# bluemoon-o2/walker-gym

Hardware: AMD Instinct MI355X
Metric: env-steps/sec (whole node) at 65 536 walkers; 1/2/4/8 MI355X scaling (higher is better)
Workload: dtype f32

## Files before the change

include/walker_hip.h:

```cpp
#ifndef WALKER_HIP_H
#define WALKER_HIP_H
#include <stdint.h>

#ifdef __cplusplus
extern "C" {
#endif

typedef struct ihipStream_t *hipStream_t;
typedef struct ihipEvent_t *hipEvent_t;

#define WG_ABI_VERSION 16
#define WG_EINVAL (-1)
#define WG_ERANGE (-2)
#define WG_EHIP (-3)

typedef struct wg_params {
    double g, dampk, ground, groundk, grounddamp, friction, dt;
    double pk, vk, ak, mk;
    int32_t in3d, max_steps;
    int32_t midform;
    int32_t conmid;
    int32_t spring_mode;
    int32_t action_mode;
    int32_t integrator;
// ... 124 lines not shown
               int32_t plan_blocks, hipStream_t stream);

typedef wg_params wg_obs_cfg;
int wg_step_simple(const wg_batch *b, const float *action, const wg_params *p, int32_t n_steps, hipStream_t stream);
int wg_observe_simple(const wg_batch *b, const wg_obs_cfg *cfg, float *obs, float *reward, uint8_t *done,
                      float *centroid, float *energy, hipStream_t stream);

int wg_reset(const wg_batch *b, const wg_params *p, const float *noise, const uint8_t *mask,
             hipStream_t stream);

int wg_reset_noise(const wg_batch *b, const float *noise, hipStream_t stream);

int wg_plan_ragged(const int32_t *mass_off, const int32_t *edge_off, const int32_t *muscle_off,
                   int32_t N, int32_t *plan, int32_t max_blocks);

int wg_plan_waves(const int32_t *mass_off, const int32_t *edge_off, const int32_t *muscle_off,
                  int32_t N, int32_t *plan, int32_t max_tiles);
int wg_wave_edge_passes(int32_t M, int32_t K);

int wg_plan_errors(int32_t clear);

int wg_launch_geometry(const wg_batch *b, wg_launch_info *info);

int wg_debug_stamps(unsigned long long *host, int n);

int wg_launch_floor(int32_t mode, int32_t blocks, int32_t threads, const float *in, float *out, int32_t n_launches,
                    hipStream_t stream);

int wg_time_step(const wg_batch *batch, const wg_params *params, const float *action, int32_t action_cols,
                 int32_t action_stride, int64_t action_step, const wg_outputs *out, int32_t n_steps,
                 const int32_t *plan, int32_t plan_blocks, hipStream_t stream, float *ms_per_launch);

#ifdef __cplusplus
}
#endif
#endif
```

walker_gym_amd/_lib.py:

```python
from __future__ import annotations

import ctypes as C
import os
import threading

HERE = os.path.dirname(os.path.abspath(__file__))
LIB_NAME = "libwalker_hip.so"
LIB_PATH = os.path.join(HERE, LIB_NAME)
ABI_VERSION = 16

WG_EINVAL, WG_ERANGE, WG_EHIP = -1, -2, -3

_vp = C.c_void_p


class WgParams(C.Structure):
    _fields_ = [(n, C.c_double) for n in ("g", "dampk", "ground", "groundk", "grounddamp", "friction", "dt",
                                           "pk", "vk", "ak", "mk")] + \
               [(n, C.c_int32) for n in ("in3d", "max_steps", "midform", "conmid", "spring_mode", "action_mode",
                                         "integrator", "pair_mode")] + \
               [(n, C.c_double) for n in ("pair_g", "pair_k", "pair_e", "bounce_k")] + \
               [("g3_gravity", C.c_double * 3)] + \
               [(n, C.c_double) for n in ("g3_damping", "g3_air", "g3_ground_level", "g3_restitution",
                                          "g3_friction")] + [("g3_ground", C.c_int32), ("friction_mode", C.c_int32),
# ... 27 lines not shown
    _fields_ = [("batch", C.POINTER(WgBatch)), ("outputs", C.POINTER(WgOutputs)), ("action_offset", C.c_int64),
                ("plan", _vp), ("plan_blocks", C.c_int32), ("stream", _vp)]


class WgLaunchInfo(C.Structure):
    _fields_ = [("threads", C.c_int32), ("walkers_per_block", C.c_int32), ("blocks", C.c_int32),
                ("lds_bytes", C.c_int32)]


class WgPolicy(C.Structure):
    _fields_ = [("n_sets", C.c_int32), ("obs_dim", C.c_int32), ("hidden", C.c_int32), ("act_dim", C.c_int32),
                ("w1", _vp), ("b1", _vp), ("w2", _vp), ("b2", _vp), ("act_limit", C.c_float),
                ("action_out", _vp), ("action_out_step", C.c_int64), ("return_out", _vp), ("length_out", _vp)]


class WgEpisodeStats(C.Structure):
    _fields_ = [("return_sum", _vp), ("length_sum", _vp), ("episodes_done", _vp), ("tail_return", _vp),
                ("tail_length", _vp), ("ep_return", _vp), ("ep_length", _vp), ("ep_slots", C.c_int32)]


EXPORTS = ("wg_abi_version", "wg_last_error", "wg_step", "wg_step_ranges", "wg_run_ranges", "wg_rollout", "wg_observe",
           "wg_step_simple", "wg_observe_simple", "wg_reset", "wg_reset_noise", "wg_plan_ragged", "wg_plan_waves",
           "wg_wave_edge_passes", "wg_plan_errors", "wg_launch_geometry", "wg_launch_floor", "wg_time_step",
           "wg_rollout_policy", "wg_rollout_episodes")

_lib = None
_lock = threading.Lock()


class WalkerHipError(RuntimeError):
    pass


def load(path: str | None = None):
    global _lib
    with _lock:
        if _lib is not None:
            return _lib
        p = path or os.environ.get("WALKER_HIP_LIB", LIB_PATH)
        if not os.path.exists(p):
            raise WalkerHipError(
                f"{p} not found: build it with `python -m walker_gym_amd.build` (hipcc --offload-arch=gfx950); "
                "walker_gym_amd has no CPU fallback")
        L = C.CDLL(p)
        L.wg_abi_version.restype = C.c_int
        L.wg_last_error.restype = C.c_char_p
        L.wg_step.argtypes = [C.POINTER(WgBatch), C.POINTER(WgParams), _vp, C.c_int32, C.c_int32, C.c_int64,
# ... 1 lines not shown
        L.wg_rollout.argtypes = L.wg_step.argtypes
        L.wg_rollout_policy.argtypes = [C.POINTER(WgBatch), C.POINTER(WgParams), C.POINTER(WgPolicy),
                                        C.POINTER(WgOutputs), C.c_int32, _vp]
        L.wg_rollout_episodes.argtypes = [C.POINTER(WgBatch), C.POINTER(WgParams), C.POINTER(WgPolicy),
                                          C.POINTER(WgOutputs), C.POINTER(WgEpisodeStats), C.c_int32, _vp]
        L.wg_step_ranges.argtypes = [C.POINTER(WgRange), C.c_int32, C.POINTER(WgParams), _vp, C.c_int32, C.c_int32,
                                     C.POINTER(_vp)]
        L.wg_run_ranges.argtypes = [C.POINTER(WgRange), C.c_int32, C.POINTER(WgParams), _vp, C.c_int32, C.c_int32,
                                    C.c_int64, C.c_int32, C.POINTER(_vp)]
        L.wg_observe.argtypes = [C.POINTER(WgBatch), C.POINTER(WgParams), C.POINTER(WgOutputs), _vp, C.c_int32, _vp]
        L.wg_step_simple.argtypes = [C.POINTER(WgBatch), _vp, C.POINTER(WgParams), C.c_int32, _vp]
        L.wg_observe_simple.argtypes = [C.POINTER(WgBatch), C.POINTER(WgParams), _vp, _vp, _vp, _vp, _vp, _vp]
        L.wg_reset.argtypes = [C.POINTER(WgBatch), C.POINTER(WgParams), _vp, _vp, _vp]
        L.wg_reset_noise.argtypes = [C.POINTER(WgBatch), _vp, _vp]
        L.wg_plan_ragged.argtypes = [_vp, _vp, _vp, C.c_int32, _vp, C.c_int32]
        L.wg_plan_waves.argtypes = [_vp, _vp, _vp, C.c_int32, _vp, C.c_int32]
        L.wg_wave_edge_passes.argtypes = [C.c_int32, C.c_int32]
        L.wg_plan_errors.argtypes = [C.c_int32]
        L.wg_launch_geometry.argtypes = [C.POINTER(WgBatch), C.POINTER(WgLaunchInfo)]
        L.wg_launch_floor.argtypes = [C.c_int32, C.c_int32, C.c_int32, _vp, _vp, C.c_int32, _vp]
        L.wg_time_step.argtypes = L.wg_step.argtypes + [C.POINTER(C.c_float)]
        for f in EXPORTS[2:]:
            getattr(L, f).restype = C.c_int
        v = L.wg_abi_version()
        if v != ABI_VERSION:
            raise WalkerHipError(f"{p}: ABI version {v}, expected {ABI_VERSION}")
        _lib = L
        return L


def check(rc: int, what: str) -> int:
    if rc < 0:
        msg = load().wg_last_error().decode(errors="replace")
        exc = ValueError if rc in (WG_EINVAL, WG_ERANGE) else WalkerHipError
        raise exc(f"{what}: {msg} (code {rc})")
    return rc
```

walker_gym_amd/csrc/walker_hip.hip:

```cpp

#include <hip/hip_runtime.h>
#include <hip/hip_ext.h>

#include <algorithm>
#include <cstdarg>
#include <cstdint>
#include <cstdio>
#include <cstdlib>
#include <cstring>
#include <type_traits>
#include <vector>

#include "walker_hip.h"
#include "powf2.h"

namespace {

thread_local char g_err[512] = "";

int fail(int code, const char *fmt, ...) __attribute__((format(printf, 2, 3)));
int fail(int code, const char *fmt, ...) {
    va_list ap;
    va_start(ap, fmt);
    vsnprintf(g_err, sizeof g_err, fmt, ap);
    va_end(ap);
    return code;
}
// ... 1567 lines not shown
    spring_terms(e, x, pix, piy, piz, pjx, pjy, pjz, vix, viy, viz, vjx, vjy, vjz, t0, t1, t2, g0, g1, g2, spring_mode,
                 pos_ok);
    ts.put(le, t0, t1, t2, g0, g1, g2);
    gt = gt || fexp3(g0, g1, g2) < TINY_EXP;
}

struct EdgeRec8 { uint32_t w; float rest; };
template <int NE, bool E8 = false>
struct LeanIn {
    float p3[3], v3[3];
    typename std::conditional<E8, EdgeRec8, EdgeRec>::type er[NE];
    uint32_t gi[NE];
    float mf;
    int io0, io1, wsteps, pin;
    float x, lo, hi, stp, a;
};

struct LeanTile {
    int w0, nw, nP, nE, nU, wl, q, mu_wl, mu_ua;
    uint32_t P0, E0, U0;
    bool is_mass, is_mus, acts;
};

__device__ __forceinline__ LeanTile lean_tile_of(const wg_batch &b, const float *action, int action_cols,
                                                 const LeanGeo &lg, int tile, int lane) {
    LeanTile t;
    t.w0 = tile * lg.wpw;
    t.nw = min(lg.wpw, b.N - t.w0);
    t.nP = t.nw * b.M; t.nE = t.nw * b.K; t.nU = t.nw * b.A;
    t.P0 = (uint32_t)t.w0 * b.M; t.E0 = (uint32_t)t.w0 * b.K; t.U0 = (uint32_t)t.w0 * b.A;
    t.wl = lane >> lg.lgM; t.q = lane & (b.M - 1);
    t.is_mass = lane < t.nP;
    t.is_mus = lane < t.nU;
    t.mu_wl = b.A > 0 ? fdiv(lane, b.A, lg.invA) : 0;
    t.mu_ua = lane - t.mu_wl * b.A;
    t.acts = action != nullptr && t.is_mus && t.mu_ua < action_cols;
    return t;
}

template <typename T>
__device__ __forceinline__ const T &at_u32(const T *base, uint32_t byte_off) {
    return *reinterpret_cast<const T *>(reinterpret_cast<const char *>(base) + (size_t)byte_off);
}
template <typename T>
__device__ __forceinline__ T &at_u32w(T *base, uint32_t byte_off) {
    return *reinterpret_cast<T *>(reinterpret_cast<char *>(base) + (size_t)byte_off);
}
#define WG_ST(base, e, n) (&at_u32w((base), (uint32_t)(n) * 4u * (uint32_t)(e)))
__device__ __forceinline__ float neg_half_count(int n) { return -0.5f * (float)n; }
template <class LI>
__device__ __forceinline__ void lean_load_mass(const wg_batch &b, const LeanTile &t, int lane, LI &L) {
    L.mf = 0.f; L.io0 = 0; L.io1 = 0; L.wsteps = 0; L.pin = 0;
    const int ln = min(lane, t.nP - 1);
    const int wl = ln >> (31 - __builtin_clz(b.M)), q = ln & (b.M - 1);
    L.mf = at_u32(b.mass, 4u * (t.P0 + ln));
    if (b.pinned) L.pin = at_u32(b.pinned, t.P0 + ln);
    const uint32_t io = (uint32_t)(t.w0 + wl) * (b.M + 1) + q;
    L.io0 = at_u32(b.inc_off, 2u * io); L.io1 = at_u32(b.inc_off, 2u * io + 2u);
    L.wsteps = at_u32(b.steps, 4u * (uint32_t)(t.w0 + wl));
}
template <class LI>
__device__ __forceinline__ void lean_load_muscles(const wg_batch &b, const KParams &kp, const float *__restrict__ action,
                                                  int action_stride, const LeanTile &t, int lane, LI &L) {
    L.x = 0.f; L.lo = 0.f; L.hi = 0.f; L.stp = 0.f; L.a = 0.f;
    if (t.nU > 0) {
        const uint32_t ul = t.U0 + min(lane, t.nU - 1);
        L.x = at_u32(b.muscle_x, 4u * ul);
        if (action && action_stride > 0) {
            const float2 bd = at_u32(reinterpret_cast<const float2 *>(b.muscle_bounds), 8u * ul);
            L.lo = bd.x; L.hi = bd.y;
            if (kp.action_mode == 1) L.stp = at_u32(b.muscle_stride, 4u * ul);
            const int wl = min(t.mu_wl, t.nw - 1), ua = max(0, min(t.mu_ua, action_stride - 1));
            L.a = at_u32(action, 4u * ((uint32_t)(t.w0 + wl) * (uint32_t)action_stride + (uint32_t)ua));
        }
    }
}
template <int NE, bool E8>
__device__ __forceinline__ void lean_load(const wg_batch &b, const KParams &kp, const float *__restrict__ action,
                                          int action_stride, const LeanTile &t, int lane, LeanIn<NE, E8> &L) {
    const uint32_t pl = t.P0 + min(lane, t.nP - 1);
    const float *gp = &at_u32(b.pos, 12u * pl), *gv = &at_u32(b.vel, 12u * pl);
    L.p3[0] = gp[0]; L.p3[1] = gp[1]; L.p3[2] = gp[2];
    L.v3[0] = gv[0]; L.v3[1] = gv[1]; L.v3[2] = gv[2];
#pragma unroll
    for (int it = 0; it < NE; it++) {
        const uint32_t le = t.E0 + (uint32_t)min(lane + 64 * it, t.nE - 1);
        if constexpr (E8) {
            const uint2 v = at_u32(reinterpret_cast<const uint2 *>(b.edges8), 8u * le);
            L.er[it] = EdgeRec8{v.x, __uint_as_float(v.y)};
        } else {
            const uint4 v = at_u32(reinterpret_cast<const uint4 *>(b.edges), 16u * le);
            L.er[it] = EdgeRec{v.x, __uint_as_float(v.y), __uint_as_float(v.z), __uint_as_float(v.w)};
        }
        L.gi[it] = at_u32(reinterpret_cast<const uint32_t *>(b.inc), 4u * le);
    }
    lean_load_mass(b, t, lane, L);
    lean_load_muscles(b, kp, action, action_stride, t, lane, L);
    if (!t.is_mass) {
        L.p3[0] = 0.f; L.p3[1] = 0.f; L.p3[2] = 0.f; L.v3[0] = 0.f; L.v3[1] = 0.f; L.v3[2] = 0.f;
        L.mf = 0.f; L.pin = 0; L.io0 = 0; L.io1 = 0;
    }
    if (!t.is_mus) { L.x = 0.f; L.lo = 0.f; L.hi = 0.f; L.stp = 0.f; }
// ... 135 lines not shown
    if (kp.pair_mode & 2) {
        const double e = (b.charge && is_mass) ? b.charge[pl] : kp.pair_e;
        pair_central(kp.pair_k, e, p3, mf, lane, M, is_mass, ax, ay, az);
    }
    if (kp.pair_mode & 4) {
        const double rs = is_mass ? b.radius[pl] : 0.0;
        const int bs = b.bounce_set ? (is_mass ? (int)b.bounce_set[pl] : 0) : 3;
        pair_bounce(kp.bounce_kh, rs, bs, p3, mf, lane, M, is_mass, ax, ay, az);
    }
    if (kp.pair_mode & 8) pair_g2_gravity(kp.pair_g, p3, mf, lane, M, is_mass, ax, ay, az);
    if (kp.pair_mode & 16) {
        const double e = (b.charge && is_mass) ? b.charge[pl] : kp.pair_e;
        pair_central(kp.pair_k, e, p3, mf, lane, M, is_mass, ax, ay, az, true);
    }
}



typedef TermsAoS LeanTerms;
__device__ __forceinline__ LeanTerms lean_terms(char *sl, const LeanGeo &lg) {
    return TermsAoS{reinterpret_cast<double *>(sl), reinterpret_cast<float *>(sl + lg.off_df)};
}

template <bool IN3D>
__device__ __forceinline__ void lean_obs_rows(float *obs, int stride, const KParams &kp, int M, int A, int w0, int wl,
                                              int q, int mu_wl, int mu_ua, bool mass_on, bool mus_on, float px, float py,
                                              float pz, float vx, float vy, float vz, float ax, float ay, float az,
                                              float sx, float sy, float sz, float midx, float midy, float midz, float x) {
    constexpr int d = IN3D ? 3 : 2, per = 3 * d;
    const int nmid = kp.conmid ? 3 : 0;
    typedef float fvd __attribute__((ext_vector_type(d), aligned(4)));
    if (mass_on) {
        const uint32_t row0 = (uint32_t)(w0 + wl) * (uint32_t)stride;
        const float mm[3] = {kp.midform == 2 ? sx : midx, kp.midform == 2 ? sy : midy, kp.midform == 2 ? sz : midz};
        const float pm[3] = {px, py, pz}, vm[3] = {vx, vy, vz}, am[3] = {ax, ay, az};
        fvd vp, vv, va;
#pragma unroll
        for (int c = 0; c < d; c++) {
            vp[c] = kp.midform ? (pm[c] - mm[c]) * kp.pk : pm[c] * kp.pk;
            vv[c] = vm[c] * kp.vk;
            va[c] = am[c] * kp.ak;
        }
        float *dst = WG_ST(obs, row0 + per * q, 1);
        *reinterpret_cast<fvd *>(dst) = vp;
        *reinterpret_cast<fvd *>(dst + d) = vv;
        *reinterpret_cast<fvd *>(dst + 2 * d) = va;
        if (q == 0) {
            if (nmid) {
                float *mrow = WG_ST(obs, row0 + per * M, 1);
                mrow[0] = kp.midform ? mm[0] : 0.f; mrow[1] = kp.midform ? mm[1] : 0.f;
                mrow[2] = kp.midform ? mm[2] : 0.f;
            }
            for (int r = per * M + nmid + A; r < stride; r++) *WG_ST(obs, row0 + r, 1) = 0.f;
        }
    }
    if (mus_on) *WG_ST(obs, (uint32_t)(w0 + mu_wl) * (uint32_t)stride + per * M + nmid + mu_ua, 1) = x * kp.mk;
}

struct LeanPolOut { float ax, ay, az, sx, sy, sz, reward; int done; int reset; };
template <bool IN3D, int NE, bool RES = false, bool E8 = false, bool AR = false, bool POL = false>
__device__ __forceinline__ void lean_compute(const wg_batch &b, const KParams &kp, const KOut &o,
                                             const LeanGeo &lg, char *sl, const LeanTile &t, int lane,
                                             LeanIn<NE, E8> &L, bool last = true, const KReset &ar = KReset{},
                                             LeanPolOut *po = nullptr, uint32_t *epw = nullptr, int epw_stride = 1) {
    const bool store = !RES || last;
    const int M = b.M, K = b.K, A = b.A;
    const int w0 = t.w0, nE = t.nE;
    const int wl = t.wl, q = t.q, mu_wl = t.mu_wl, mu_ua = t.mu_ua;
    const bool is_mass = t.is_mass, is_mus = t.is_mus, acts = t.acts;
    const uint32_t pl = t.P0 + lane, ul = t.U0 + lane;
    const LeanTerms ts = lean_terms(sl, lg);
#ifdef WG_STAMPS
    const int stamp_wave = t.w0 / lg.wpw;
#endif
    uint32_t *s_inc = reinterpret_cast<uint32_t *>(sl + lg.off_inc);
    float *s_x = reinterpret_cast<float *>(sl + lg.off_x);
    const float mf = L.mf;
    const bool pin = L.pin != 0;
    double sq_tl = 0.0, sq_te = 0.0;
    if (NE == 1 && !RES) {
        sq_tl = PW_LOG2_TAB[lane & 31];
        sq_te = pw_asdouble(PW_EXP2_TAB[lane & 31]);
    }

    if (!RES) {
#pragma unroll
        for (int it = 0; it < NE; it++)
            if (lane + 64 * it < nE) s_inc[lane + 64 * it] = L.gi[it];
        if (lane == 0) s_inc[nE] = 0u;
    }
    float x = L.x;
    if (acts) {
        x = (kp.action_mode == 1) ? ((L.a != 0.f) ? x + L.stp : x - L.stp) : x + L.a;
        if (L.lo > x) x = L.lo;
        if (L.hi < x) x = L.hi;
        if (store) *WG_ST(b.muscle_x, ul, 1) = x;
    }
    if (is_mus) s_x[lane] = x;
    double ym = recip_m(mf);
    if (!RES) asm volatile("" : "+v"(ym));
    wave_sync();
    STAMP(2);

    bool dead = false;
    if ((!RES || NE == 1) && kp.pair_mode == 0) {
        const bool nanp = is_mass && (__builtin_isnan(L.p3[0]) || __builtin_isnan(L.p3[1]) || __builtin_isnan(L.p3[2]));
        if (__builtin_expect(__ballot(nanp) != 0ull, 0)) {
            const unsigned long long db = __ballot(nanp && !pin && L.io1 > L.io0);
            const unsigned long long gm = (M == 64) ? ~0ull : (((1ull << M) - 1ull) << (lane & ~(M - 1)));
            dead = is_mass && (db & gm) == gm;
            if (dead) {
// ... 24 lines not shown
                continue;
            }
            g.v[c] = lane_gather(L.p3[c], bi); g.v[3 + c] = lane_gather(L.p3[c], bj);
            g.v[6 + c] = lane_gather(L.v3[c], bi); g.v[9 + c] = lane_gather(L.v3[c], bj);
        }
    };
    auto spring = [&](int it, const Gath &g) {
        const int le = lane + 64 * it;
        EdgeRec e;
        float xr;
        if constexpr (E8) {
            const uint32_t w = L.er[it].w;
            const bool mus = (w & 0x40000000u) != 0u;
            const float xs = *reinterpret_cast<const float *>(reinterpret_cast<const char *>(s_x) + ((w >> 16) & 0xfcu));
            xr = mus ? xs : L.er[it].rest;
            e = EdgeRec{w, L.er[it].rest, mus ? b.kc[0] : b.kc[2], mus ? b.kc[1] : b.kc[3]};
        } else {
            e = L.er[it];
            const int ewl = fdiv(le, K, lg.invK), ew = le - (int)__umul24(ewl, K);
            const bool mus = le < nE && ew < A;
            const float xs = s_x[mus ? (int)__umul24(ewl, A) + ew : 0];
            xr = mus ? xs : e.rest;
        }
        if (le < nE) {
            if (WG_ABLATE & 1) {
                ts.put(le, xr + g.v[0] + g.v[3] + g.v[6] + g.v[9], g.v[1] + g.v[4] + g.v[7] + g.v[10],
                       g.v[2] + g.v[5] + g.v[8] + g.v[11], e.k, e.c, 0.f);
            } else {
                spring_edge_regs(e, le, xr, g.v[0], g.v[1], g.v[2], g.v[3], g.v[4], g.v[5], g.v[6], g.v[7], g.v[8],
                                 g.v[9], g.v[10], g.v[11], ts, 0, gtiny, pos_ok);
            }
        }
    };
#pragma unroll
    for (int it = 0; it < NE; it++) {
        if (64 * it >= nE) continue;
        if ((WG_ABLATE & 4096) && it == NE - 1 && it > 0) {
            const int le = lane + 64 * it;
            if (le < nE) ts.put(le, 0.0, 0.0, 0.0, 0.f, 0.f, 0.f);
            continue;
        }
        Gath g;
        gather(it, g);
        spring(it, g);
    }
    wave_sync();
    const bool wave_tiny = __any(gtiny);
    STAMP(3);

    EnvTerms et{};
    if (!RES) et = env_terms(kp, mf, (float)ym, L.v3[0], L.v3[1], L.v3[2]);
    float px = 0.f, py = 0.f, pz = 0.f, vx = 0.f, vy = 0.f, vz = 0.f, ax = 0.f, ay = 0.f, az = 0.f;
    float nv = 0.f, ke = 0.f, pe = 0.f;
    bool hit = false;
    if (is_mass) {
        const int r1 = (WG_ABLATE & 2) ? min(L.io1, L.io0 + 1) : L.io1;
        const int lb = wl * K;
        if (!RES)
            mass_accumulate_v2(ts, reinterpret_cast<const uint16_t *>(s_inc) + 2 * lb, lb, L.io0, r1, mf, ym, ax, ay, az,
                               wave_tiny);
        else
            mass_accumulate<LeanTerms, !RES>(ts, reinterpret_cast<const uint16_t *>(s_inc) + 2 * lb, lb, L.io0, r1, mf,
                                             ax, ay, az, 0, wave_tiny);
    }
    if (!RES && kp.pair_mode) pair_forces(b, kp, L.p3, mf, pl, lane, M, is_mass, ax, ay, az);
    if (is_mass) {
        mass_tail(kp, mf, (float)ym, L.p3, L.v3, px, py, pz, vx, vy, vz, ax, ay, az, hit, pin,
                  !RES ? &et : nullptr);
        if (dead) {
            px = __builtin_nanf(""); py = px; pz = px; vx = px; vy = px; vz = px; ax = px; ay = px; az = px;
            hit = false;
        }
        if (b.radius && store) b.radius[pl] = hit ? 3.0 : 1.0;
        nv = np_norm3(vx, vy, vz);
        if (!(NE == 1 && !RES)) ke = dead ? nv : mf * np_sq<NE == 1>(nv);
        pe = (float)((double)mf * kp.g) * (py - kp.ground);
    }
    if (NE == 1 && !RES) {
        const float sq = np_sq_wave(dead ? 0.f : nv, sq_tl, sq_te);
        if (is_mass) ke = dead ? nv : mf * sq;
    }
    STAMP(4);

    const int gbase = lane & ~(M - 1);
    const WalkerSums ws = (WG_ABLATE & 4) ? WalkerSums{px, py, pz, py, nv, ke, pe}
                                          : walker_sums(px, py, pz, nv, ke, pe, gbase, M, lane);
    const float sx = ws.sx, sy = ws.sy, sz = ws.sz, ysum = ws.ysum, vsum = ws.vsum, ksum = ws.ksum, psum = ws.psum;
    const unsigned long long gmask = (M == 64) ? ~0ull : (((1ull << M) - 1ull) << gbase);
    const unsigned long long hb = __ballot(is_mass && (py - kp.ground < 0.f));
    const unsigned long long sb = __ballot(is_mass && nv < 0.1f);
    const float midx = sx * lg.invM, midy = sy * lg.invM, midz = sz * lg.invM;
    int ep_done = 0;
    if (is_mass) {
        if (store) {
            float *gpo = WG_ST(b.pos, pl, 3), *gvo = WG_ST(b.vel, pl, 3), *gao = WG_ST(b.acc, pl, 3);
            gpo[0] = px; gpo[1] = py; gpo[2] = pz;
            gvo[0] = vx; gvo[1] = vy; gvo[2] = vz;
            if (RES || kp.keep_aux) {
                gao[0] = ax; gao[1] = ay; gao[2] = az;
                if (b.contact) at_u32w(b.contact, pl) = (uint8_t)hit;
            }
        }
        if (q == 0) {
            const uint32_t wg = (uint32_t)(w0 + wl);
            const int steps = L.wsteps + 1;
            if (store) *WG_ST(b.steps, wg, 1) = steps;
            if (RES) L.wsteps = steps;
            if (o.steps) *WG_ST(o.steps, wg, 1) = steps;
            const float cy = ysum * lg.invM;
            if constexpr (POL) {
                const float vpen = (-(vsum * lg.invM)) * 0.1f;
                po->reward = (cy + vpen) + neg_half_count((int)__popcll(hb & gmask));
                if (o.reward) *WG_ST(o.reward, wg, 1) = po->reward;
            } else if (o.reward) {
                const float vpen = (-(vsum * lg.invM)) * 0.1f;
                *WG_ST(o.reward, wg, 1) = (cy + vpen) + neg_half_count((int)__popcll(hb & gmask));
            }
            if (o.done || (AR && (ar.mode & 1)) || POL) {
                int done = steps >= kp.max_steps;
                if (!done && cy < kp.done_y) done = 1;
                if (!done && steps > 100) done = (sb & gmask) == gmask;
                if (o.done) at_u32w(o.done, wg) = (uint8_t)done;
                ep_done = done;
            }
            if (o.centroid) {
                float *c = WG_ST(o.centroid, wg, 3);
                c[0] = midx; c[1] = midy; c[2] = midz;
            }
            if (o.energy) *WG_ST(o.energy, wg, 1) = 0.5f * ksum + psum;
        }
    }

    STAMP(5);
    if (o.obs && !(WG_ABLATE & 16))
        lean_obs_rows<IN3D>(o.obs, o.obs_stride, kp, M, A, w0, wl, q, mu_wl, mu_ua, is_mass, is_mus, px, py, pz, vx, vy,
                            vz, ax, ay, az, sx, sy, sz, midx, midy, midz, x);
    float rsx = sx, rsy = sy, rsz = sz;
    if constexpr (AR) {
        const bool nonf = is_mass && !(__builtin_isfinite(px) && __builtin_isfinite(py) && __builtin_isfinite(pz) &&
                                       __builtin_isfinite(vx) && __builtin_isfinite(vy) && __builtin_isfinite(vz) &&
                                       __builtin_isfinite(ax) && __builtin_isfinite(ay) && __builtin_isfinite(az));
        const unsigned long long eb = __ballot(is_mass && q == 0 && ep_done != 0), nb = __ballot(nonf);
        const unsigned long long hot = ((ar.mode & 1) ? eb : 0ull) | ((ar.mode & 2) ? nb : 0ull);
        const bool selw = is_mass && (hot & gmask) != 0ull;
        if (ar.reset && is_mass && q == 0) at_u32w(ar.reset, (uint32_t)(w0 + wl)) = (uint8_t)selw;
        if constexpr (POL) po->reset = selw;
        if (__builtin_expect(hot != 0ull, 0)) {
            const unsigned long long mmask = (M == 64) ? ~0ull : (((1ull << M) - 1ull) << ((mu_wl << lg.lgM) & 63));
            const bool selm = is_mus && (hot & mmask) != 0ull;
            if (ar.final_obs)
                lean_obs_rows<IN3D>(ar.final_obs, o.obs_stride, kp, M, A, w0, wl, q, mu_wl, mu_ua, selw, selm, px, py, pz,
                                    vx, vy, vz, ax, ay, az, sx, sy, sz, midx, midy, midz, x);
            int ep = 0;
            if (selw && q == 0) ep = RES ? (int)epw[wl * epw_stride] : at_u32(b.episodes, 4u * (uint32_t)(w0 + wl));
            ep = __builtin_amdgcn_ds_bpermute(gbase << 2, ep);
            float fx = px, fy = py, fz = pz, fvx = vx, fvy = vy, fvz = vz, fax = ax, fay = ay, faz = az, fxm = x;
            if (selw) {
                const float *ip = &at_u32(b.init_pos, 12u * pl), *iv = &at_u32(b.init_vel, 12u * pl),
                            *ia = &at_u32(b.init_acc, 12u * pl);
// ... 45 lines not shown
    }
    if (RES) {
        L.p3[0] = px; L.p3[1] = py; L.p3[2] = pz;
        L.v3[0] = vx; L.v3[1] = vy; L.v3[2] = vz;
        L.x = x;
    }
    if constexpr (POL) {
        po->ax = ax; po->ay = ay; po->az = az;
        po->sx = rsx; po->sy = rsy; po->sz = rsz;
        po->done = ep_done;
    }
    STAMP(6);
#ifdef WG_STAMPS
    if (lane == 0 && stamp_wave < (1 << 16)) {
        const unsigned hw = __builtin_amdgcn_s_getreg((31 << 11) | 4);
        const unsigned xcc = __builtin_amdgcn_s_getreg((31 << 11) | 20);
        g_stamps[stamp_wave * 8 + 7] = (unsigned long long)hw | ((unsigned long long)xcc << 32);
    }
#endif
}

constexpr int lean_waves(int NE) { return NE >= 8 ? 4 : 6; }

template <bool IN3D, int NE, bool E8, bool AR = false>
__global__ __launch_bounds__(256) __attribute__((amdgpu_waves_per_eu(lean_waves(NE)))) void walker_step_lean(
    typename std::conditional<AR, wg_batch, KBatch15>::type bk, KParams kp, const float *__restrict__ action,
    int action_cols, int action_stride, KOut o, LeanGeo lg, typename std::conditional<AR, KReset, KNoReset>::type ar) {
    extern __shared__ __attribute__((aligned(16))) char smem[];
    const wg_batch b = batch_of(bk);
    const int lane = threadIdx.x & 63, wv = __builtin_amdgcn_readfirstlane(threadIdx.x >> 6);
    const int blk = (kp.xcd & 2) ? xcd_block(blockIdx.x, gridDim.x) : (int)blockIdx.x;
    const int tile = blk * lg.wpb + wv;
    if (tile * lg.wpw >= b.N) return;
#ifdef WG_STAMPS
    const int stamp_wave = tile;
#endif
    STAMP(0);
    const LeanTile t = lean_tile_of(b, action, action_cols, lg, tile, lane);
    LeanIn<NE, E8> L;
    if (kp.prio) __builtin_amdgcn_s_setprio(2);
    lean_load<NE, E8>(b, kp, action, action_stride, t, lane, L);
    if (kp.prio) __builtin_amdgcn_s_setprio(0);
    STAMP(1);
    if constexpr (AR) lean_compute<IN3D, NE, false, E8, true>(b, kp, o, lg, smem + wv * lg.slice, t, lane, L, true, ar);
    else lean_compute<IN3D, NE, false, E8>(b, kp, o, lg, smem + wv * lg.slice, t, lane, L);
}

template <bool IN3D, bool E8, bool AR = false>
__global__ __launch_bounds__(256) __attribute__((amdgpu_waves_per_eu(lean_waves(1)))) void walker_step_lean1(
    float *pos, float *vel, const void *edges, const uint16_t *inc, int N, int M, int K, int wpw, int wpb, int nblkx,
    wg_batch b, KParams kp, const float *__restrict__ action, int action_cols, int action_stride, KOut o, LeanGeo lg,
    typename std::conditional<AR, KReset, KNoReset>::type ar) {
    extern __shared__ __attribute__((aligned(16))) char smem[];
    b.pos = pos; b.vel = vel; b.inc = inc; b.N = N; b.M = M; b.K = K;
    if (E8) b.edges8 = static_cast<const wg_edge8 *>(edges);
    else b.edges = static_cast<const wg_edge *>(edges);
    lg.nblk = nblkx & 0x3fffffff; lg.wpw = wpw; lg.wpb = wpb;
    kp.prio = (int)((unsigned)nblkx >> 31);
    const int lane = threadIdx.x & 63, wv = __builtin_amdgcn_readfirstlane(threadIdx.x >> 6);
    const int bid = blockIdx.x, xb = xcd_block(bid, lg.nblk);
    const int blk = (nblkx & 0x40000000) ? xb : bid;
    const int tile = blk * lg.wpb + wv;
    if (tile * lg.wpw >= b.N) return;
#ifdef WG_STAMPS
    const int stamp_wave = tile;
#endif
    STAMP(0);
    const LeanTile t = lean_tile_of(b, action, action_cols, lg, tile, lane);
    LeanIn<1, E8> L;
    if (kp.prio) __builtin_amdgcn_s_setprio(2);
    lean_load<1, E8>(b, kp, action, action_stride, t, lane, L);
    if (kp.prio) __builtin_amdgcn_s_setprio(0);
    STAMP(1);
    if constexpr (AR) lean_compute<IN3D, 1, false, E8, true>(b, kp, o, lg, smem + wv * lg.slice, t, lane, L, true, ar);
    else lean_compute<IN3D, 1, false, E8>(b, kp, o, lg, smem + wv * lg.slice, t, lane, L);
}

struct KResetRes {
    KReset r;
    int off_ep;
};
__device__ __forceinline__ KReset kreset_at(const KReset &r, const KOut &o, int s) {
    KReset as = r;
    if (as.reset) as.reset += (size_t)s * o.out_step;
    if (as.final_obs) as.final_obs += (size_t)s * o.obs_step;
    return as;
}
template <bool IN3D, int NE, bool E8, bool AR = false>
__global__ __launch_bounds__(256) __attribute__((amdgpu_waves_per_eu(NE >= 8 ? 4 : 5))) void walker_rollout_lean(
    wg_batch b, KParams kp, const float *__restrict__ action, int action_cols, int action_stride, int64_t action_step,
    KOut o, int n_steps, LeanGeo lg, typename std::conditional<AR, KResetRes, KNoReset>::type ar) {
    extern __shared__ __attribute__((aligned(16))) char smem[];
    const int lane = threadIdx.x & 63, wv = __builtin_amdgcn_readfirstlane(threadIdx.x >> 6);
    const int tile = blockIdx.x * lg.wpb + wv;
    if (tile * lg.wpw >= b.N) return;
#ifdef WG_STAMPS
    const int stamp_wave = tile;
#endif
// ... 797 lines not shown
    if (wcap > 0 && wcap < g.wpw) g.wpw = wcap;
    g.lgM = 0;
    while ((1 << g.lgM) < M) g.lgM++;
    if ((g.wpw * b->K + 63) / 64 > 8 || g.wpw * b->A > 64) return false;
    const int wpb = env_int("WG_LEAN_WAVES", 0);
    g.wpb = (wpb == 1 || wpb == 2 || wpb == 4) ? wpb : ((b->N + g.wpw - 1) / g.wpw <= 1024 ? 1 : 4);
    const int ew = g.wpw * b->K;
    g.pl = (ew + 3) & ~3;
    g.off_df = align16(g.pl * 24);
    g.off_inc = g.off_df + align16(g.pl * 12);
    g.off_x = g.off_inc + align16(ew * 4 + 4);
    g.slice = g.off_x + align16(std::max(1, g.wpw * b->A) * 4);
    if (4 * g.slice > 80 * 1024) return false;
    g.invK = 1.f / (float)b->K;
    g.invA = 1.f / (float)std::max(1, b->A);
    g.invM = 1.f / (float)M;
    g.nblk = (b->N + g.wpb * g.wpw - 1) / (g.wpb * g.wpw);
    *out = g;
    return true;
}

int lean_blocks(const wg_batch *b, const LeanGeo &g) { return (b->N + g.wpb * g.wpw - 1) / (g.wpb * g.wpw); }

int launch_lean(const wg_batch *b, const KParams &kp, bool in3d, const float *a, int cols, int astride,
                const wg_outputs &o, const LeanGeo &g, hipStream_t st, int ar_mode = 0) {
    const int blocks = lean_blocks(b, g);
    const int ne = (g.wpw * b->K + 63) / 64;
    const int lds = g.wpb * g.slice + std::max(0, env_int("WG_LDS_PAD", 0));
    const bool e8 = use_edge8(b, g);
#define WG_LAUNCH_LEAN(D3, NE_, E8_)                                                                             \
    do {                                                                                                         \
        if (ar_mode)                                                                                             \
            WG_KLAUNCH((walker_step_lean<D3, NE_, E8_, true>), dim3(blocks), dim3(64 * g.wpb), (uint32_t)lds,    \
                       st, *b, kp, a, cols, astride, kout(o), g, kreset(o, ar_mode));                            \
        else                                                                                                     \
            WG_KLAUNCH((walker_step_lean<D3, NE_, E8_>), dim3(blocks), dim3(64 * g.wpb), (uint32_t)lds, st,      \
                       kbatch15(b), kp, a, cols, astride, kout(o), g, KNoReset{});                               \
    } while (0)
#define WG_LEAN_NE(D3, E8_)                                                    \
    do {                                                                       \
        if (ne == 2) WG_LAUNCH_LEAN(D3, 2, E8_);                               \
        else if (ne == 3) WG_LAUNCH_LEAN(D3, 3, E8_);                          \
        else if (ne == 4) WG_LAUNCH_LEAN(D3, 4, E8_);                          \
        else WG_LAUNCH_LEAN(D3, 8, E8_);                                       \
    } while (0)
#define WG_LEAN1_ARGS(E8_)                                                                                       \
    b->pos, b->vel, (E8_) ? static_cast<const void *>(b->edges8) : static_cast<const void *>(b->edges), b->inc,  \
        b->N, b->M, b->K, g.wpw, g.wpb,                                                                          \
        (int)((unsigned)g.nblk | ((unsigned)(kp.xcd & 2) << 29) | ((unsigned)(kp.prio != 0) << 31)), *b, kp, a,  \
        cols, astride, kout(o), g
#define WG_LAUNCH_LEAN1(D3, E8_)                                                                                 \
    do {                                                                                                         \
// ... 545 lines not shown
    for (int i = 0; i < n_launches; i++) {
        if (mode == 0)
            hipLaunchKernelGGL(floor_empty_kernel, dim3(blocks), dim3(threads), 0, stream, out);
        else if (mode == 1)
            hipLaunchKernelGGL(floor_load_store_kernel, dim3(blocks), dim3(threads), 0, stream, in, out);
        else
            hipLaunchKernelGGL(floor_busy_kernel, dim3(blocks), dim3(threads), 0, stream, in, out);
    }
    return hipGetLastError() == hipSuccess ? 0 : fail(WG_EHIP, "floor launch failed");
}

int wg_debug_stamps(unsigned long long *host, int n) {
#ifdef WG_STAMPS
    if (hipMemcpyFromSymbol(host, HIP_SYMBOL(g_stamps), (size_t)n * 8 * sizeof(unsigned long long), 0,
                            hipMemcpyDeviceToHost) != hipSuccess)
        return fail(WG_EHIP, "stamp copy failed");
    return 0;
#else
    (void)host; (void)n;
    return fail(WG_EINVAL, "not a stamps build");
#endif
}

int wg_launch_geometry(const wg_batch *b, wg_launch_info *info) {
    int rc = validate(b);
    if (rc) return rc;
    if (!info) return fail(WG_EINVAL, "null info");
    LeanGeo lg{};
    if (lean_geo(b, 0, &lg)) {
        info->threads = 64 * lg.wpb;
        info->walkers_per_block = lg.wpb * lg.wpw;
        info->blocks = lean_blocks(b, lg);
        info->lds_bytes = lg.wpb * lg.slice;
        return 0;
    }
    RagGeo rg{};
    if (b->ragged == 2 && lean_enabled() && rag_geo(b, 0, &rg)) {
        info->threads = 64 * rg.wpb;
        info->walkers_per_block = -1;
        info->blocks = -1;
        info->lds_bytes = rg.wpb * rg.slice;
        return 0;
    }
    const Geo g = b->ragged ? ragged_geo(b) : uniform_geo(b, 0);
    info->threads = g.threads;
    info->walkers_per_block = g.W;
// ... 7 lines not shown
```

walker_gym_amd/device.py:

```python
from __future__ import annotations

import ctypes as C
import os
from typing import Optional

import numpy as np
import torch

from . import _lib
from .layout import HostLayout, default_radius, refresh_edges8, set_springs


def _to_dev(a: np.ndarray, device) -> torch.Tensor:
    a = np.ascontiguousarray(a)
    if a.dtype == np.uint16:
        t = torch.from_numpy(a.view(np.int16))
    elif a.dtype == np.uint32:
        t = torch.from_numpy(a.view(np.int32))
    else:
        t = torch.from_numpy(a)
    return t.to(device, non_blocking=False).contiguous()


def _ptr(t: Optional[torch.Tensor]):
# ... 200 lines not shown
            mass=off(self.mass, M * w0), edges=off(self.edges, 4 * K * w0),
            inc=off(self.inc, 2 * K * w0) if self.inc is not None else None,
            inc_off=off(self.inc_off, (M + 1) * w0),
            muscle_x=self._p(self.muscle_x) if A == 0 else off(self.muscle_x, A * w0),
            muscle_bounds=self._p(self.muscle_bounds) if A == 0 else off(self.muscle_bounds, 2 * A * w0),
            muscle_stride=self._p(self.muscle_stride) if A == 0 else off(self.muscle_stride, A * w0),
            steps=off(self.steps, w0), contact=off(self.contact, M * w0), pinned=off(self.pinned, M * w0),
            charge=off(self.charge, M * w0), radius=off(self.radius, M * w0), row=None,
            bounce_set=off(self.bounce_set, M * w0),
            edges8=off(self.edges8, 2 * K * w0) if self.edges8 is not None and w0 % (64 // M) == 0 else None,
            kc=(C.c_float * 4)(*self.kc), **self._auto_reset_fields(w0))

    def launch_geometry(self) -> dict:
        info = _lib.WgLaunchInfo()
        _lib.check(_lib.load().wg_launch_geometry(C.byref(self.struct), C.byref(info)), "wg_launch_geometry")
        blocks = info.blocks
        if self.ragged:
            wpb = max(1, info.threads // 64)
            blocks = -(-self.plan_blocks // wpb) if self.ragged_kind == 2 else self.plan_blocks
        geo = dict(threads=info.threads, walkers_per_block=info.walkers_per_block, blocks=blocks,
                   lds_bytes=info.lds_bytes)
        if self.ragged_kind == 2:
            geo["wave_tiles"] = self.plan_blocks
        return geo

    KIND = {"pos": "mass", "vel": "mass", "acc": "mass", "contact": "mass", "radius": "mass", "muscle_x": "muscle",
            "steps": "walker"}

    def state_dict(self) -> dict:
        sd = {k: self.caller(k).clone() for k in self.STATE}
        if self.radius is not None:
            sd["radius"] = self.caller("radius").clone()
        return sd

    def load_state_dict(self, sd: dict) -> None:
        self.version += 1
        for k in self.STATE:
            getattr(self, k).copy_(self.to_stored(self.KIND[k], sd[k].to(self.device)))
        if "radius" in sd:
            self.enable_radius()
            self.radius.copy_(self.to_stored("mass", sd["radius"].to(self.device)))
```

Baseline: 2.135 billion.

## Add specialized lean step kernel for fixed default parameter configuration

Result: faster. 2.172 billion, median of 6 (+1.8%).

```diff
diff --git a/include/walker_hip.h b/include/walker_hip.h
--- a/include/walker_hip.h
+++ b/include/walker_hip.h
@@ -170,6 +170,8 @@
 
 int wg_launch_geometry(const wg_batch *b, wg_launch_info *info);
 
+long long wg_fix_launches(void);
+
 int wg_debug_stamps(unsigned long long *host, int n);
 
 int wg_launch_floor(int32_t mode, int32_t blocks, int32_t threads, const float *in, float *out, int32_t n_launches,
diff --git a/walker_gym_amd/_lib.py b/walker_gym_amd/_lib.py
--- a/walker_gym_amd/_lib.py
+++ b/walker_gym_amd/_lib.py
@@ -73,7 +73,7 @@
 EXPORTS = ("wg_abi_version", "wg_last_error", "wg_step", "wg_step_ranges", "wg_run_ranges", "wg_rollout", "wg_observe",
            "wg_step_simple", "wg_observe_simple", "wg_reset", "wg_reset_noise", "wg_plan_ragged", "wg_plan_waves",
            "wg_wave_edge_passes", "wg_plan_errors", "wg_launch_geometry", "wg_launch_floor", "wg_time_step",
-           "wg_rollout_policy", "wg_rollout_episodes")
+           "wg_rollout_policy", "wg_rollout_episodes", "wg_fix_launches")
 
 _lib = None
 _lock = threading.Lock()
@@ -121,6 +121,7 @@
         L.wg_time_step.argtypes = L.wg_step.argtypes + [C.POINTER(C.c_float)]
         for f in EXPORTS[2:]:
             getattr(L, f).restype = C.c_int
+        L.wg_fix_launches.restype = C.c_longlong
         v = L.wg_abi_version()
         if v != ABI_VERSION:
             raise WalkerHipError(f"{p}: ABI version {v}, expected {ABI_VERSION}")
diff --git a/walker_gym_amd/csrc/walker_hip.hip b/walker_gym_amd/csrc/walker_hip.hip
--- a/walker_gym_amd/csrc/walker_hip.hip
+++ b/walker_gym_amd/csrc/walker_hip.hip
@@ -3,6 +3,7 @@
 #include <hip/hip_ext.h>
 
 #include <algorithm>
+#include <atomic>
 #include <cstdarg>
 #include <cstdint>
 #include <cstdio>
@@ -1616,19 +1617,20 @@
     bool is_mass, is_mus, acts;
 };
 
+template <bool FIX = false>
 __device__ __forceinline__ LeanTile lean_tile_of(const wg_batch &b, const float *action, int action_cols,
                                                  const LeanGeo &lg, int tile, int lane) {
     LeanTile t;
     t.w0 = tile * lg.wpw;
-    t.nw = min(lg.wpw, b.N - t.w0);
+    t.nw = FIX ? lg.wpw : min(lg.wpw, b.N - t.w0);
     t.nP = t.nw * b.M; t.nE = t.nw * b.K; t.nU = t.nw * b.A;
     t.P0 = (uint32_t)t.w0 * b.M; t.E0 = (uint32_t)t.w0 * b.K; t.U0 = (uint32_t)t.w0 * b.A;
     t.wl = lane >> lg.lgM; t.q = lane & (b.M - 1);
-    t.is_mass = lane < t.nP;
+    t.is_mass = FIX || lane < t.nP;
     t.is_mus = lane < t.nU;
-    t.mu_wl = b.A > 0 ? fdiv(lane, b.A, lg.invA) : 0;
+    t.mu_wl = (FIX || b.A > 0) ? fdiv(lane, b.A, lg.invA) : 0;
     t.mu_ua = lane - t.mu_wl * b.A;
-    t.acts = action != nullptr && t.is_mus && t.mu_ua < action_cols;
+    t.acts = FIX ? t.is_mus : action != nullptr && t.is_mus && t.mu_ua < action_cols;
     return t;
 }
 
@@ -1670,8 +1672,44 @@
     }
 }
 template <int NE, bool E8>
+__device__ __forceinline__ void lean_load_fix(const wg_batch &b, const float *__restrict__ action, int action_stride,
+                                              const LeanTile &t, int lane, LeanIn<NE, E8> &L) {
+    static_assert(E8, "the fixed-parameter instance reads the compact spring records");
+    const uint32_t ln = (uint32_t)lane;
+    const float *gp = &at_u32(b.pos + 3 * (size_t)t.P0, 12u * ln), *gv = &at_u32(b.vel + 3 * (size_t)t.P0, 12u * ln);
+    L.p3[0] = gp[0]; L.p3[1] = gp[1]; L.p3[2] = gp[2];
+    L.v3[0] = gv[0]; L.v3[1] = gv[1]; L.v3[2] = gv[2];
+    const uint2 *ge = reinterpret_cast<const uint2 *>(b.edges8) + t.E0;
+    const uint32_t *gi = reinterpret_cast<const uint32_t *>(b.inc) + t.E0;
+#pragma unroll
+    for (int it = 0; it < NE; it++) {
+        const uint32_t le = it < NE - 1 ? ln + 64u * it : (uint32_t)min(lane + 64 * it, t.nE - 1);
+        const uint2 v = at_u32(ge, 8u * le);
+        L.er[it] = EdgeRec8{v.x, __uint_as_float(v.y)};
+        L.gi[it] = at_u32(gi, 4u * le);
+    }
+    L.mf = at_u32(b.mass + t.P0, 4u * ln);
+    L.pin = 0;
+    const uint32_t io = (uint32_t)t.wl * (b.M + 1) + t.q;
+    const uint16_t *go = b.inc_off + (size_t)t.w0 * (b.M + 1);
+    L.io0 = at_u32(go, 2u * io); L.io1 = at_u32(go, 2u * io + 2u);
+    L.wsteps = at_u32(b.steps + t.w0, 4u * (uint32_t)t.wl);
+    L.x = 0.f; L.lo = 0.f; L.hi = 0.f; L.stp = 0.f; L.a = 0.f;
+    if (t.is_mus) {
+        L.x = at_u32(b.muscle_x + t.U0, 4u * ln);
+        const float2 bd = at_u32(reinterpret_cast<const float2 *>(b.muscle_bounds) + t.U0, 8u * ln);
+        L.lo = bd.x; L.hi = bd.y;
+        L.a = at_u32(action + (size_t)t.w0 * (size_t)action_stride,
+                     4u * ((uint32_t)t.mu_wl * (uint32_t)action_stride + (uint32_t)t.mu_ua));
+    }
+}
+template <int NE, bool E8, bool FIX = false>
 __device__ __forceinline__ void lean_load(const wg_batch &b, const KParams &kp, const float *__restrict__ action,
                                           int action_stride, const LeanTile &t, int lane, LeanIn<NE, E8> &L) {
+    if constexpr (FIX) {
+        lean_load_fix<NE, E8>(b, action, action_stride, t, lane, L);
+        return;
+    }
     const uint32_t pl = t.P0 + min(lane, t.nP - 1);
     const float *gp = &at_u32(b.pos, 12u * pl), *gv = &at_u32(b.vel, 12u * pl);
     L.p3[0] = gp[0]; L.p3[1] = gp[1]; L.p3[2] = gp[2];
@@ -1853,24 +1891,29 @@
     return TermsAoS{reinterpret_cast<double *>(sl), reinterpret_cast<float *>(sl + lg.off_df)};
 }
 
-template <bool IN3D>
+template <bool IN3D, bool FIX = false>
 __device__ __forceinline__ void lean_obs_rows(float *obs, int stride, const KParams &kp, int M, int A, int w0, int wl,
                                               int q, int mu_wl, int mu_ua, bool mass_on, bool mus_on, float px, float py,
                                               float pz, float vx, float vy, float vz, float ax, float ay, float az,
                                               float sx, float sy, float sz, float midx, float midy, float midz, float x) {
     constexpr int d = IN3D ? 3 : 2, per = 3 * d;
-    const int nmid = kp.conmid ? 3 : 0;
+    const int nmid = (!FIX && kp.conmid) ? 3 : 0;
     typedef float fvd __attribute__((ext_vector_type(d), aligned(4)));
     if (mass_on) {
         const uint32_t row0 = (uint32_t)(w0 + wl) * (uint32_t)stride;
-        const float mm[3] = {kp.midform == 2 ? sx : midx, kp.midform == 2 ? sy : midy, kp.midform == 2 ? sz : midz};
+        const bool sums = !FIX && kp.midform == 2;
+        const float mm[3] = {sums ? sx : midx, sums ? sy : midy, sums ? sz : midz};
         const float pm[3] = {px, py, pz}, vm[3] = {vx, vy, vz}, am[3] = {ax, ay, az};
         fvd vp, vv, va;
 #pragma unroll
         for (int c = 0; c < d; c++) {
-            vp[c] = kp.midform ? (pm[c] - mm[c]) * kp.pk : pm[c] * kp.pk;
-            vv[c] = vm[c] * kp.vk;
-            va[c] = am[c] * kp.ak;
+            if constexpr (FIX) {
+                vp[c] = pm[c] - mm[c]; vv[c] = vm[c]; va[c] = am[c];
+            } else {
+                vp[c] = kp.midform ? (pm[c] - mm[c]) * kp.pk : pm[c] * kp.pk;
+                vv[c] = vm[c] * kp.vk;
+                va[c] = am[c] * kp.ak;
+            }
         }
         float *dst = WG_ST(obs, row0 + per * q, 1);
         *reinterpret_cast<fvd *>(dst) = vp;
@@ -1885,20 +1928,29 @@
             for (int r = per * M + nmid + A; r < stride; r++) *WG_ST(obs, row0 + r, 1) = 0.f;
         }
     }
-    if (mus_on) *WG_ST(obs, (uint32_t)(w0 + mu_wl) * (uint32_t)stride + per * M + nmid + mu_ua, 1) = x * kp.mk;
-}
-
+    if (mus_on)
+        *WG_ST(obs, (uint32_t)(w0 + mu_wl) * (uint32_t)stride + per * M + nmid + mu_ua, 1) = FIX ? x : x * kp.mk;
+}
+
+__device__ __forceinline__ KParams lean_fix_params(KParams kp) {
+    kp.pk = 1.f; kp.vk = 1.f; kp.ak = 1.f; kp.mk = 1.f;
+    kp.midform = 1; kp.conmid = 0; kp.action_mode = 0; kp.integrator = 0; kp.pair_mode = 0;
+    return kp;
+}
 struct LeanPolOut { float ax, ay, az, sx, sy, sz, reward; int done; int reset; };
-template <bool IN3D, int NE, bool RES = false, bool E8 = false, bool AR = false, bool POL = false>
-__device__ __forceinline__ void lean_compute(const wg_batch &b, const KParams &kp, const KOut &o,
+template <bool IN3D, int NE, bool RES = false, bool E8 = false, bool AR = false, bool POL = false, bool FIX = false>
+__device__ __forceinline__ void lean_compute(const wg_batch &b, const KParams &kp_in, const KOut &o,
                                              const LeanGeo &lg, char *sl, const LeanTile &t, int lane,
                                              LeanIn<NE, E8> &L, bool last = true, const KReset &ar = KReset{},
                                              LeanPolOut *po = nullptr, uint32_t *epw = nullptr, int epw_stride = 1) {
+    static_assert(!FIX || (E8 && !RES && !AR && !POL && NE <= 4), "FIX: the plain E8 step instance");
+    const KParams kp_fix = FIX ? lean_fix_params(kp_in) : KParams{};
+    const KParams &kp = FIX ? kp_fix : kp_in;
     const bool store = !RES || last;
     const int M = b.M, K = b.K, A = b.A;
     const int w0 = t.w0, nE = t.nE;
     const int wl = t.wl, q = t.q, mu_wl = t.mu_wl, mu_ua = t.mu_ua;
-    const bool is_mass = t.is_mass, is_mus = t.is_mus, acts = t.acts;
+    const bool is_mass = FIX || t.is_mass, is_mus = t.is_mus, acts = FIX ? t.is_mus : t.acts;
     const uint32_t pl = t.P0 + lane, ul = t.U0 + lane;
     const LeanTerms ts = lean_terms(sl, lg);
 #ifdef WG_STAMPS
@@ -1907,7 +1959,7 @@
     uint32_t *s_inc = reinterpret_cast<uint32_t *>(sl + lg.off_inc);
     float *s_x = reinterpret_cast<float *>(sl + lg.off_x);
     const float mf = L.mf;
-    const bool pin = L.pin != 0;
+    const bool pin = !FIX && L.pin != 0;
     double sq_tl = 0.0, sq_te = 0.0;
     if (NE == 1 && !RES) {
         sq_tl = PW_LOG2_TAB[lane & 31];
@@ -1917,7 +1969,7 @@
     if (!RES) {
 #pragma unroll
         for (int it = 0; it < NE; it++)
-            if (lane + 64 * it < nE) s_inc[lane + 64 * it] = L.gi[it];
+            if ((FIX && it < NE - 1) || lane + 64 * it < nE) s_inc[lane + 64 * it] = L.gi[it];
         if (lane == 0) s_inc[nE] = 0u;
     }
     float x = L.x;
@@ -1988,7 +2040,7 @@
             const float xs = s_x[mus ? (int)__umul24(ewl, A) + ew : 0];
             xr = mus ? xs : e.rest;
         }
-        if (le < nE) {
+        if ((FIX && it < NE - 1) || le < nE) {
             if (WG_ABLATE & 1) {
                 ts.put(le, xr + g.v[0] + g.v[3] + g.v[6] + g.v[9], g.v[1] + g.v[4] + g.v[7] + g.v[10],
                        g.v[2] + g.v[5] + g.v[8] + g.v[11], e.k, e.c, 0.f);
@@ -2000,7 +2052,7 @@
     };
 #pragma unroll
     for (int it = 0; it < NE; it++) {
-        if (64 * it >= nE) continue;
+        if (!FIX && 64 * it >= nE) continue;
         if ((WG_ABLATE & 4096) && it == NE - 1 && it > 0) {
             const int le = lane + 64 * it;
             if (le < nE) ts.put(le, 0.0, 0.0, 0.0, 0.f, 0.f, 0.f);
@@ -2037,7 +2089,7 @@
             px = __builtin_nanf(""); py = px; pz = px; vx = px; vy = px; vz = px; ax = px; ay = px; az = px;
             hit = false;
         }
-        if (b.radius && store) b.radius[pl] = hit ? 3.0 : 1.0;
+        if (!FIX && b.radius && store) b.radius[pl] = hit ? 3.0 : 1.0;
         nv = np_norm3(vx, vy, vz);
         if (!(NE == 1 && !RES)) ke = dead ? nv : mf * np_sq<NE == 1>(nv);
         pe = (float)((double)mf * kp.g) * (py - kp.ground);
@@ -2078,29 +2130,29 @@
                 const float vpen = (-(vsum * lg.invM)) * 0.1f;
                 po->reward = (cy + vpen) + neg_half_count((int)__popcll(hb & gmask));
                 if (o.reward) *WG_ST(o.reward, wg, 1) = po->reward;
-            } else if (o.reward) {
+            } else if (FIX || o.reward) {
                 const float vpen = (-(vsum * lg.invM)) * 0.1f;
                 *WG_ST(o.reward, wg, 1) = (cy + vpen) + neg_half_count((int)__popcll(hb & gmask));
             }
-            if (o.done || (AR && (ar.mode & 1)) || POL) {
+            if (FIX || o.done || (AR && (ar.mode & 1)) || POL) {
                 int done = steps >= kp.max_steps;
                 if (!done && cy < kp.done_y) done = 1;
                 if (!done && steps > 100) done = (sb & gmask) == gmask;
-                if (o.done) at_u32w(o.done, wg) = (uint8_t)done;
+                if (FIX || o.done) at_u32w(o.done, wg) = (uint8_t)done;
                 ep_done = done;
             }
-            if (o.centroid) {
+            if (FIX || o.centroid) {
                 float *c = WG_ST(o.centroid, wg, 3);
                 c[0] = midx; c[1] = midy; c[2] = midz;
             }
-            if (o.energy) *WG_ST(o.energy, wg, 1) = 0.5f * ksum + psum;
+            if (FIX || o.energy) *WG_ST(o.energy, wg, 1) = 0.5f * ksum + psum;
         }
     }
 
     STAMP(5);
-    if (o.obs && !(WG_ABLATE & 16))
-        lean_obs_rows<IN3D>(o.obs, o.obs_stride, kp, M, A, w0, wl, q, mu_wl, mu_ua, is_mass, is_mus, px, py, pz, vx, vy,
-                            vz, ax, ay, az, sx, sy, sz, midx, midy, midz, x);
+    if ((FIX || o.obs) && !(WG_ABLATE & 16))
+        lean_obs_rows<IN3D, FIX>(o.obs, o.obs_stride, kp, M, A, w0, wl, q, mu_wl, mu_ua, is_mass, is_mus, px, py, pz,
+                                 vx, vy, vz, ax, ay, az, sx, sy, sz, midx, midy, midz, x);
     float rsx = sx, rsy = sy, rsz = sz;
     if constexpr (AR) {
         const bool nonf = is_mass && !(__builtin_isfinite(px) && __builtin_isfinite(py) && __builtin_isfinite(pz) &&
@@ -2192,7 +2244,7 @@
 
 constexpr int lean_waves(int NE) { return NE >= 8 ? 4 : 6; }
 
-template <bool IN3D, int NE, bool E8, bool AR = false>
+template <bool IN3D, int NE, bool E8, bool AR = false, bool FIX = false>
 __global__ __launch_bounds__(256) __attribute__((amdgpu_waves_per_eu(lean_waves(NE)))) void walker_step_lean(
     typename std::conditional<AR, wg_batch, KBatch15>::type bk, KParams kp, const float *__restrict__ action,
     int action_cols, int action_stride, KOut o, LeanGeo lg, typename std::conditional<AR, KReset, KNoReset>::type ar) {
@@ -2206,17 +2258,17 @@
     const int stamp_wave = tile;
 #endif
     STAMP(0);
-    const LeanTile t = lean_tile_of(b, action, action_cols, lg, tile, lane);
+    const LeanTile t = lean_tile_of<FIX>(b, action, action_cols, lg, tile, lane);
     LeanIn<NE, E8> L;
     if (kp.prio) __builtin_amdgcn_s_setprio(2);
-    lean_load<NE, E8>(b, kp, action, action_stride, t, lane, L);
+    lean_load<NE, E8, FIX>(b, kp, action, action_stride, t, lane, L);
     if (kp.prio) __builtin_amdgcn_s_setprio(0);
     STAMP(1);
     if constexpr (AR) lean_compute<IN3D, NE, false, E8, true>(b, kp, o, lg, smem + wv * lg.slice, t, lane, L, true, ar);
-    else lean_compute<IN3D, NE, false, E8>(b, kp, o, lg, smem + wv * lg.slice, t, lane, L);
-}
-
-template <bool IN3D, bool E8, bool AR = false>
+    else lean_compute<IN3D, NE, false, E8, false, false, FIX>(b, kp, o, lg, smem + wv * lg.slice, t, lane, L);
+}
+
+template <bool IN3D, bool E8, bool AR = false, bool FIX = false>
 __global__ __launch_bounds__(256) __attribute__((amdgpu_waves_per_eu(lean_waves(1)))) void walker_step_lean1(
     float *pos, float *vel, const void *edges, const uint16_t *inc, int N, int M, int K, int wpw, int wpb, int nblkx,
     wg_batch b, KParams kp, const float *__restrict__ action, int action_cols, int action_stride, KOut o, LeanGeo lg,
@@ -2236,14 +2288,14 @@
     const int stamp_wave = tile;
 #endif
     STAMP(0);
-    const LeanTile t = lean_tile_of(b, action, action_cols, lg, tile, lane);
+    const LeanTile t = lean_tile_of<FIX>(b, action, action_cols, lg, tile, lane);
     LeanIn<1, E8> L;
     if (kp.prio) __builtin_amdgcn_s_setprio(2);
-    lean_load<1, E8>(b, kp, action, action_stride, t, lane, L);
+    lean_load<1, E8, FIX>(b, kp, action, action_stride, t, lane, L);
     if (kp.prio) __builtin_amdgcn_s_setprio(0);
     STAMP(1);
     if constexpr (AR) lean_compute<IN3D, 1, false, E8, true>(b, kp, o, lg, smem + wv * lg.slice, t, lane, L, true, ar);
-    else lean_compute<IN3D, 1, false, E8>(b, kp, o, lg, smem + wv * lg.slice, t, lane, L);
+    else lean_compute<IN3D, 1, false, E8, false, false, FIX>(b, kp, o, lg, smem + wv * lg.slice, t, lane, L);
 }
 
 struct KResetRes {
@@ -3087,12 +3139,58 @@
 
 int lean_blocks(const wg_batch *b, const LeanGeo &g) { return (b->N + g.wpb * g.wpw - 1) / (g.wpb * g.wpw); }
 
+bool lean_fix_ok(const wg_batch *b, const KParams &kp, const float *a, int cols, int astride, const wg_outputs &o,
+                 const LeanGeo &g, bool e8, int ne, int ar_mode) {
+#ifdef WG_STAMPS
+    return false;
+#endif
+    if (WG_ABLATE != 0 || env_int("WG_FIX", 1) == 0) return false;
+    auto one = [](float f) {
+        uint32_t u;
+        memcpy(&u, &f, sizeof u);
+        return u == 0x3f800000u;
+    };
+    return e8 && ne >= 1 && ne <= 4 && ar_mode == 0 && b->N % g.wpw == 0 && g.wpw * b->M == 64 &&
+           b->A >= 1 && a != nullptr && cols >= b->A && astride >= b->A && kp.action_mode == 0 &&
+           kp.pair_mode == 0 && !b->pinned && !b->radius && kp.integrator != 2 && kp.midform == 1 && kp.conmid == 0 &&
+           one(kp.pk) && one(kp.vk) && one(kp.ak) && one(kp.mk) &&
+           o.obs && o.reward && o.done && o.centroid && o.energy;
+}
+std::atomic<long long> g_fix_launches{0};
+
 int launch_lean(const wg_batch *b, const KParams &kp, bool in3d, const float *a, int cols, int astride,
                 const wg_outputs &o, const LeanGeo &g, hipStream_t st, int ar_mode = 0) {
     const int blocks = lean_blocks(b, g);
     const int ne = (g.wpw * b->K + 63) / 64;
     const int lds = g.wpb * g.slice + std::max(0, env_int("WG_LDS_PAD", 0));
     const bool e8 = use_edge8(b, g);
+    if (lean_fix_ok(b, kp, a, cols, astride, o, g, e8, ne, ar_mode)) {
+#define WG_LAUNCH_FIX(D3, NE_)                                                                                   \
+    WG_KLAUNCH((walker_step_lean<D3, NE_, true, false, true>), dim3(blocks), dim3(64 * g.wpb), (uint32_t)lds, st, \
+               kbatch15(b), kp, a, cols, astride, kout(o), g, KNoReset{})
+#define WG_LAUNCH_FIX1(D3)                                                                                       \
+    WG_KLAUNCH((walker_step_lean1<D3, true, false, true>), dim3(blocks), dim3(64 * g.wpb), (uint32_t)lds, st,    \
+               b->pos, b->vel, static_cast<const void *>(b->edges8), b->inc, b->N, b->M, b->K, g.wpw, g.wpb,     \
+               (int)((unsigned)g.nblk | ((unsigned)(kp.xcd & 2) << 29) | ((unsigned)(kp.prio != 0) << 31)), *b,  \
+               kp, a, cols, astride, kout(o), g, KNoReset{})
+        if (in3d) {
+            if (ne == 1) WG_LAUNCH_FIX1(true);
+            else if (ne == 2) WG_LAUNCH_FIX(true, 2);
+            else if (ne == 3) WG_LAUNCH_FIX(true, 3);
+            else WG_LAUNCH_FIX(true, 4);
+        } else {
+            if (ne == 1) WG_LAUNCH_FIX1(false);
+            else if (ne == 2) WG_LAUNCH_FIX(false, 2);
+            else if (ne == 3) WG_LAUNCH_FIX(false, 3);
+            else WG_LAUNCH_FIX(false, 4);
+        }
+#undef WG_LAUNCH_FIX1
+#undef WG_LAUNCH_FIX
+        const hipError_t ef = hipGetLastError();
+        if (ef != hipSuccess) return fail(WG_EHIP, "launch failed: %s", hipGetErrorString(ef));
+        g_fix_launches.fetch_add(1, std::memory_order_relaxed);
+        return 0;
+    }
 #define WG_LAUNCH_LEAN(D3, NE_, E8_)                                                                             \
     do {                                                                                                         \
         if (ar_mode)                                                                                             \
@@ -3684,6 +3782,8 @@
 #endif
 }
 
+long long wg_fix_launches(void) { return g_fix_launches.load(std::memory_order_relaxed); }
+
 int wg_launch_geometry(const wg_batch *b, wg_launch_info *info) {
     int rc = validate(b);
     if (rc) return rc;
diff --git a/walker_gym_amd/device.py b/walker_gym_amd/device.py
--- a/walker_gym_amd/device.py
+++ b/walker_gym_amd/device.py
@@ -246,6 +246,7 @@
                    lds_bytes=info.lds_bytes)
         if self.ragged_kind == 2:
             geo["wave_tiles"] = self.plan_blocks
+        geo["fix_launches"] = int(_lib.load().wg_fix_launches())
         return geo
 
     KIND = {"pos": "mass", "vel": "mass", "acc": "mass", "contact": "mass", "radius": "mass", "muscle_x": "muscle",
```
